# mks0601/ExAvatar_RELEASE

Measured on NVIDIA H100. Metric: avatar train-step frames/sec (fwd+bwd raster), higher is better.
Workload: dtype f32

## Files before the change

### exavatar_release_b200/csrc/composite_bwd4.cu

```cuda
#include "common.cuh"

namespace b2r {

constexpr int B4_THREADS = 64;
constexpr int B4_BATCH = 64;
#ifndef B4_QUEUE_DEPTH
#define B4_QUEUE_DEPTH 16
#endif
#ifndef B4_MIN_BLOCKS
#define B4_MIN_BLOCKS 10
#endif
constexpr int B4_QUEUE = B4_QUEUE_DEPTH;

struct B4Stage {
  float4 a[B4_BATCH];
  float4 b[B4_BATCH];
  float4 c[B4_BATCH];
};
constexpr int B4_GROUP = 4;
constexpr int B4_CQ = 32 + B4_GROUP;
struct B4Compact {
  float4 r[3][B4_CQ];
};
static_assert(B4_QUEUE % B4_GROUP == 0, "phase B runs when whole groups fill the transposition queue");

__device__ __forceinline__ float rcp_approx4(float x) {
  float y;
  asm("rcp.approx.ftz.f32 %0, %1;" : "=f"(y) : "f"(x));
  return y;
}

struct B4Smem {
  B4Stage stage[2];
  B4Compact compact[2];
  float2 tb[2][B4_QUEUE][33];
  float4 qm0[2][B4_QUEUE];
  float4 qm1[2][B4_QUEUE];
  float4 gpix[2][32];
  int warp_max_s[2];
};

template <bool HAS_DA>
__device__ __forceinline__ void bwd4_item(const B2RScene& sc, const Ctx& cx, const B2RBackwardArgs& args,
                                          float* __restrict__ gacc, B4Smem& sm, const int t_pos, const int seg,
                                          const int quad, const int n_multi) {
  B4Stage (&stage)[2] = sm.stage;
  B4Compact (&compact)[2] = sm.compact;
  float2 (&tb)[2][B4_QUEUE][33] = sm.tb;
  float4 (&qm0)[2][B4_QUEUE] = sm.qm0;
  float4 (&qm1)[2][B4_QUEUE] = sm.qm1;
  float4 (&gpix)[2][32] = sm.gpix;
  int (&warp_max_s)[2] = sm.warp_max_s;
  B2R_TRACE_BEGIN();
  const bool multi = t_pos < n_multi;
  const int tile = (int)cx.tile_order[t_pos];
  if (cx.skip_below && cx.tile_maxid[tile] < cx.skip_below) return;
  const int tx = tile % cx.gx, ty = tile / cx.gx;
  const int lane = threadIdx.x & 31, warp = threadIdx.x >> 5;
  const int W = sc.width, H = sc.height;
  const int wx0 = tx * TILE + (quad & 1) * 8, wy0 = ty * TILE + (quad >> 1) * 8 + warp * 4;
  if (wx0 >= W || ty * TILE + (quad >> 1) * 8 >= H) return;
  const int px = wx0 + (lane & 7), py = wy0 + (lane >> 3);
  const bool inside = px < W && py < H;
  const float pxf = (float)px, pyf = (float)py;
  const float rx0 = (float)wx0, ry0 = (float)wy0;
  const float rx1 = fminf((float)(wx0 + 7), (float)(W - 1)), ry1 = fminf((float)(wy0 + 3), (float)(H - 1));
  const size_t N = (size_t)W * H;
  const size_t pix = (size_t)py * W + px;

  const uint2 range = cx.ranges[tile];
  const int n = (int)(range.y - range.x);
  const int lo = multi ? seg * SEG : 0;
  const int hi = multi ? min(n, lo + SEG) : n;
  const uint32_t* ids = cx.dup_ids + range.x + lo;

  const int my_n = inside ? (int)cx.n_contrib[pix] : 0;
  const int my_hi = min(my_n, hi) - lo;
  const bool cont = my_n > hi;
  const float T_final = inside ? cx.final_T[pix] : 0.f;
  const float g_r = inside ? __ldg(args.dL_dcolor + pix) : 0.f;
  const float g_g = inside ? __ldg(args.dL_dcolor + N + pix) : 0.f;
  const float g_b = inside ? __ldg(args.dL_dcolor + 2 * N + pix) : 0.f;
  float g_d = 0.f, g_a = 0.f;
  if (HAS_DA && inside) {
    if (args.dL_ddepth) g_d = __ldg(args.dL_ddepth + pix);
    if (args.dL_dalpha) g_a = __ldg(args.dL_dalpha + pix);
  }
  const float* bgp = cx.bg ? cx.bg : sc.bg;
  const float Tfb = T_final * (__ldg(bgp) * g_r + __ldg(bgp + 1) * g_g + __ldg(bgp + 2) * g_b);
  gpix[warp][lane] = make_float4(g_r, g_g, g_b, g_d);

  const int warp_n = __reduce_max_sync(0xffffffffu, max(my_hi, 0));
  if (lane == 0) warp_max_s[warp] = warp_n;
  __syncthreads();
  const int nmax = max(warp_max_s[0], warp_max_s[1]);
  if (nmax == 0) {
    B2R_TRACE_END(0);
    return;
  }
  const int nb = (nmax + B4_BATCH - 1) / B4_BATCH;

  float T = T_final, B = 0.f;
  if (cont) {
    const int pit = (py - ty * TILE) * TILE + (px - tx * TILE);
    const int nrec = (n + SEG - 1) / SEG;
    const float* rec = cx.ckpt + (size_t)(cx.seg_start[t_pos] + seg) * CK_REC_FLOATS;
    const float* fin = cx.ckpt + (size_t)(cx.seg_start[t_pos] + nrec - 1) * CK_REC_FLOATS;
    const float4 c = __ldg(reinterpret_cast<const float4*>(rec) + pit);
    const float4 f = __ldg(reinterpret_cast<const float4*>(fin) + pit);
    float num = (f.y - c.y) * g_r + (f.z - c.z) * g_g + (f.w - c.w) * g_b;
    if (HAS_DA) {
      const float2 c2 = __ldg(reinterpret_cast<const float2*>(rec + CK_PLANE0) + pit);
      const float2 f2 = __ldg(reinterpret_cast<const float2*>(fin + CK_PLANE0) + pit);
      num += (f2.x - c2.x) * g_d + (f2.y - c2.y) * g_a;
    }
    T = c.x;
    B = __fdividef(num, c.x);
  }
  float la = 0.f, olm = 1.f, lv = 0.f;
  int qpos = 0;
  B4Compact& cw = compact[warp];
  const bool lane0 = lane == 0;
  const unsigned lanes_above = 0xfffffffeu << lane;
  const uint32_t first_grad = args.first_row;

  auto drain = [&](const int count) {
    constexpr int SHARE = 32 / B4_QUEUE;
    constexpr int ROWS = 4 / SHARE;
    static_assert(B4_QUEUE == 8 || B4_QUEUE == 16 || B4_QUEUE == 32, "queue depth");
    __syncwarp();
    const int h = lane & (B4_QUEUE - 1), part = lane / B4_QUEUE;
    const bool live = h < count;
    float Sx = 0.f, Sy = 0.f, Sxx = 0.f, Sxy = 0.f, Syy = 0.f, Sq = 0.f, Sr = 0.f, Sg = 0.f, Sb = 0.f, Sd = 0.f;
    float4 m0 = make_float4(0.f, 0.f, 0.f, 0.f), m1 = make_float4(0.f, 1.f, 0.f, 0.f);
    if (live) {
      m0 = qm0[warp][h];
      m1 = qm1[warp][h];
      const float mx = m0.x - rx0, my = m0.y - ry0;
      float dxs[8];
#pragma unroll
      for (int c = 0; c < 8; c++) dxs[c] = mx - (float)c;
#pragma unroll
      for (int r = 0; r < ROWS; r++) {
        const float dy = my - (float)(part * ROWS + r);
        float Rq = 0.f, Rx = 0.f, Rxx = 0.f;
#pragma unroll
        for (int c = 0; c < 8; c++) {
          const int p = (part * ROWS + r) * 8 + c;
          const float2 t = tb[warp][h][p];
          const float4 g = gpix[warp][p];
          const float hx = t.x * dxs[c];
          Rq += t.x;
          Rx += hx;
          Rxx = fmaf(hx, dxs[c], Rxx);
          Sr = fmaf(t.y, g.x, Sr);
          Sg = fmaf(t.y, g.y, Sg);
          Sb = fmaf(t.y, g.z, Sb);
          if (HAS_DA) Sd = fmaf(t.y, g.w, Sd);
        }
        const float hy = Rq * dy;
        Sq += Rq;
        Sx += Rx;
        Sxx += Rxx;
        Sy += hy;
        Syy = fmaf(hy, dy, Syy);
        Sxy = fmaf(Rx, dy, Sxy);
      }
    }
#pragma unroll
    for (int o = B4_QUEUE; o < 32; o <<= 1) {
      Sx += __shfl_xor_sync(0xffffffffu, Sx, o);
      Sy += __shfl_xor_sync(0xffffffffu, Sy, o);
      Sxx += __shfl_xor_sync(0xffffffffu, Sxx, o);
      Sxy += __shfl_xor_sync(0xffffffffu, Sxy, o);
      Syy += __shfl_xor_sync(0xffffffffu, Syy, o);
      Sq += __shfl_xor_sync(0xffffffffu, Sq, o);
      Sr += __shfl_xor_sync(0xffffffffu, Sr, o);
      Sg += __shfl_xor_sync(0xffffffffu, Sg, o);
      Sb += __shfl_xor_sync(0xffffffffu, Sb, o);
      if (HAS_DA) Sd += __shfl_xor_sync(0xffffffffu, Sd, o);
    }
    const uint32_t gid = __float_as_uint(m1.z) & 0x1fffffffu;
    if (live && part == 0 && gid >= first_grad) {
      float* dst = gacc + (size_t)gid * 12;
      red_add_v4(dst, 2.f * m0.z * Sx + m0.w * Sy, 2.f * m1.x * Sy + m0.w * Sx, Sxx, Sxy);
      red_add_v4(dst + 4, Syy, __fdividef(Sq, m1.y), Sd, 0.f);
      red_add_v4(dst + 8, Sr, Sg, Sb, 0.f);
    }
    __syncwarp();
  };

  const uint32_t id_begin = cx.id_begin, id_span = cx.id_span;
  uint32_t next_id = 0u;
  auto prefetch = [&](int b) {
    const int idx = b * B4_BATCH + threadIdx.x;
    next_id = idx < nmax ? __ldg(ids + idx) : 0u;
  };
  auto issue = [&](int b) {
    B4Stage& s = stage[b & 1];
    const int idx = b * B4_BATCH + threadIdx.x;
    if (idx < nmax) {
      const uint32_t id = next_id;
      if (id - id_begin < id_span) {
        const float4* src = reinterpret_cast<const float4*>(cx.geom + id);
        cp_async16(&s.a[threadIdx.x], src);
        cp_async16(&s.b[threadIdx.x], src + 1);
        cp_async16(&s.c[threadIdx.x], src + 2);
      } else {
        s.a[threadIdx.x] = make_float4(0.f, 0.f, -1.f, 0.f);
        s.b[threadIdx.x] = make_float4(-1.f, 0.f, 0.f, INFINITY);
      }
    }
    cp_async_commit();
  };

  auto replay_group = [&](const int k) {
    float araw[B4_GROUP], vv[B4_GROUP];
    bool valid[B4_GROUP];
#pragma unroll
    for (int u = 0; u < B4_GROUP; u++) {
      const float4 a = cw.r[0][k + u], bb = cw.r[1][k + u], col = cw.r[2][k + u];
      const float dx = a.x - pxf, dy = a.y - pyf;
      const float p2 = a.z * dx * dx + bb.x * dy * dy + a.w * dx * dy;
      araw[u] = bb.y * ex2_approx(p2);
      valid[u] = (__float_as_int(bb.w) < my_hi) && (p2 <= 0.f) && (araw[u] >= K_ALPHA_MIN);
      float v = fmaf(col.z, g_b, fmaf(col.y, g_g, col.x * g_r));
      if (HAS_DA) v += fmaf(bb.z, g_d, g_a);
      vv[u] = v;
      if (lane0) {
        qm0[warp][qpos + u] = a;
        qm1[warp][qpos + u] = make_float4(bb.x, bb.y, col.w, 0.f);
      }
    }
#pragma unroll
    for (int u = 0; u < B4_GROUP; u++) {
      const float ae = valid[u] ? fminf(K_ALPHA_MAX, araw[u]) : 0.f;
      const float om = 1.f - ae;
      const float rcp = rcp_approx4(om);
      const float Tn = T * rcp;
      B = fmaf(la, lv, olm * B);
      const float dLda = fmaf(vv[u] - B, Tn, -Tfb * rcp);
      la = ae; olm = om; lv = vv[u]; T = Tn;
      tb[warp][qpos + u][lane] = make_float2(valid[u] ? araw[u] * dLda : 0.f, ae * Tn);
    }
    qpos += B4_GROUP;
    if (qpos == B4_QUEUE) {
      drain(B4_QUEUE);
      qpos = 0;
    }
  };

  int head = 0, fill = 0;
  prefetch(nb - 1);
  issue(nb - 1);
  if (nb > 1) prefetch(nb - 2);
  for (int b = nb - 1; b >= 0; b--) {
    cp_async_wait<0>();
    __syncthreads();
    if (b > 0) {
      issue(b - 1);
      if (b > 1) prefetch(b - 2);
    }
    const int count = min(B4_BATCH, nmax - b * B4_BATCH);
    const B4Stage& s = stage[b & 1];
    if (warp_n <= b * B4_BATCH) continue;
    for (int c0 = ((count - 1) >> 5) << 5; c0 >= 0; c0 -= 32) {
      const int idx = c0 + lane;
      const int pos = b * B4_BATCH + idx;
      bool hit = false;
      float4 a, bb;
      if (idx < count && pos < warp_n) {
        a = s.a[idx];
        bb = s.b[idx];
        hit = !(region_max_p2(a.x, a.y, a.z, a.w, bb.x, rx0, ry0, rx1, ry1) < bb.w);
      }
      const unsigned mask = __ballot_sync(0xffffffffu, hit);
      if (mask == 0u) continue;
      if (hit) {
        int slot = head + fill + __popc(mask & lanes_above);
        slot -= slot >= B4_CQ ? B4_CQ : 0;
        cw.r[0][slot] = a;
        cw.r[1][slot] = make_float4(bb.x, bb.y, bb.z, __int_as_float(pos));
        cw.r[2][slot] = s.c[idx];
      }
      fill += __popc(mask);
      __syncwarp();
      for (; fill >= B4_GROUP; fill -= B4_GROUP) {
        replay_group(head);
        head = head + B4_GROUP == B4_CQ ? 0 : head + B4_GROUP;
      }
      __syncwarp();
    }
  }
  if (fill > 0) {
    if (lane >= fill && lane < B4_GROUP) {
      cw.r[0][head + lane] = make_float4(0.f, 0.f, 0.f, 0.f);
      cw.r[1][head + lane] = make_float4(0.f, 1.f, 0.f, __int_as_float(0x7fffffff));
      cw.r[2][head + lane] = make_float4(0.f, 0.f, 0.f, 0.f);
    }
    __syncwarp();
    replay_group(head);
  }
  if (qpos > 0) drain(qpos);
  if (threadIdx.x == 0) atomicAdd(reinterpret_cast<unsigned long long*>(&cx.status->consumed_bwd), (unsigned long long)nmax);
  B2R_TRACE_END(nmax);
}

template <bool HAS_DA>
__global__ void __launch_bounds__(B4_THREADS, B4_MIN_BLOCKS) composite_bwd4_kernel(const B2RScene sc, const Ctx cx,
                                                                    const B2RBackwardArgs args, float* __restrict__ gacc) {
  __shared__ B4Smem sm;
  const int n_multi = cx.ckpt ? (int)cx.classes[CLS_N_MULTI] : 0;
  const int total_segs = cx.ckpt ? (int)cx.classes[CLS_TOTAL_SEGS] : 0;
  const int items = 4 * (total_segs + (cx.tiles - n_multi));
  for (int item = blockIdx.x; item < items; item += gridDim.x) {
    const int s_item = item >> 2;
    int t_pos, seg;
    if (s_item < total_segs) {
      const uint2 e = cx.seg_table[s_item];
      t_pos = (int)e.x;
      seg = (int)e.y;
    } else {
      t_pos = n_multi + (s_item - total_segs);
      seg = 0;
    }
    bwd4_item<HAS_DA>(sc, cx, args, gacc, sm, t_pos, seg, item & 3, n_multi);
    __syncthreads();
  }
}

int launch_composite_bwd(const B2RScene& sc, const Ctx& cx, const B2RBackwardArgs& a, float* gacc, cudaStream_t st) {
  if (!(a.flags & B2R_BWD_SCRATCH_ZEROED)) cudaMemsetAsync(gacc, 0, (size_t)(sc.P > 0 ? sc.P : 1) * 12 * sizeof(float), st);
  const uint64_t extra = cx.ckpt ? cx.dup_capacity / SEG : 0;
  const uint64_t bound = 4ull * ((uint64_t)cx.tiles + extra);
  const uint64_t cap = (uint64_t)device_sm_count() * B4_MIN_BLOCKS * 4;
  const unsigned grid = (unsigned)(bound < cap ? bound : cap);
  ProfScope p(K_COMPOSITE_BWD, st);
  if (a.dL_ddepth || a.dL_dalpha)
    launch_k(composite_bwd4_kernel<true>, grid, B4_THREADS, 0, st, false, sc, cx, a, gacc);
  else
    launch_k(composite_bwd4_kernel<false>, grid, B4_THREADS, 0, st, false, sc, cx, a, gacc);
  return check_launch();
}

}

#ifdef B2R_CTA_TRACE
extern "C" int b2r_debug_trace_bwd(unsigned long long* buf) {
  return (int)cudaMemcpyToSymbol(b2r::g_cta_trace, &buf, sizeof(buf));
}
#endif
```

### exavatar_release_b200/csrc/composite_fwd4.cu

```cuda
#include "common.cuh"

namespace b2r {

#ifndef FL_BATCH_N
#define FL_BATCH_N 128
#endif
constexpr int F4_BATCH = 2 * FL_BATCH_N;
#ifndef F4_GROUP_N
#define F4_GROUP_N 4
#endif
constexpr int F4_GROUP = F4_GROUP_N;
constexpr int F4_CQ = 32 + F4_GROUP;

struct F4Stage {
  float4 a[F4_BATCH];
  float4 b[F4_BATCH];
  float4 c[F4_BATCH];
};
struct F4Queue {
  float4 r[3][F4_CQ];
};
struct Blend {
  float T, Tf, Cr, Cg, Cb, Dp, Aa;
  uint32_t last;
};
__device__ __forceinline__ bool alive(const Blend& s) { return s.T >= K_T_MIN; }

__device__ __forceinline__ void store4v(float* base, bool vec_ok, int lane, float v, bool inside) {
  if (vec_ok) {
    const float v1 = __shfl_down_sync(0xffffffffu, v, 1);
    const float v2 = __shfl_down_sync(0xffffffffu, v, 2);
    const float v3 = __shfl_down_sync(0xffffffffu, v, 3);
    if ((lane & 3) == 0 && inside) *reinterpret_cast<float4*>(base) = make_float4(v, v1, v2, v3);
  } else if (inside) {
    *base = v;
  }
}

__device__ __forceinline__ void blend_group4(const F4Queue& cw, const int k, Blend& s, const float pxf, const float pyf) {
  float al[F4_GROUP], om[F4_GROUP];
  bool ok[F4_GROUP];
  float4 col[F4_GROUP];
  float dep[F4_GROUP];
  uint32_t pos[F4_GROUP];
#pragma unroll
  for (int u = 0; u < F4_GROUP; u++) {
    const float4 a = cw.r[0][k + u], bb = cw.r[1][k + u];
    col[u] = cw.r[2][k + u];
    const float dx = a.x - pxf, dy = a.y - pyf;
    const float p2 = a.z * dx * dx + bb.x * dy * dy + a.w * dx * dy;
    const float ar = bb.y * ex2_approx(p2);
    al[u] = fminf(K_ALPHA_MAX, ar);
    ok[u] = (ar >= K_ALPHA_MIN) & (p2 <= 0.f);
    om[u] = ok[u] ? 1.f - al[u] : 1.f;
    dep[u] = bb.z;
    pos[u] = (uint32_t)__float_as_int(bb.w);
  }
#pragma unroll
  for (int u = 0; u < F4_GROUP; u++) {
    const float w = al[u] * s.T;
    const float Tn = s.T * om[u];
    const bool use = ok[u] & (Tn >= K_T_MIN);
    s.Cr = use ? fmaf(col[u].x, w, s.Cr) : s.Cr;
    s.Cg = use ? fmaf(col[u].y, w, s.Cg) : s.Cg;
    s.Cb = use ? fmaf(col[u].z, w, s.Cb) : s.Cb;
    s.Dp = use ? fmaf(dep[u], w, s.Dp) : s.Dp;
    s.Aa = use ? s.Aa + w : s.Aa;
    s.last = use ? pos[u] : s.last;
    s.Tf = use ? Tn : s.Tf;
    s.T = Tn;
  }
}

__device__ __forceinline__ void cull_and_blend(const F4Stage& st, const int idx, const bool in_range, const int pos1,
                                               F4Queue& cw, int& head, int& fill, Blend& s, const float rx0, const float ry0,
                                               const float rx1, const float ry1, const float pxf, const float pyf) {
  const int lane = threadIdx.x & 31;
  bool hit = false;
  float4 a, bb;
  if (in_range) {
    a = st.a[idx];
    bb = st.b[idx];
    hit = !(region_max_p2(a.x, a.y, a.z, a.w, bb.x, rx0, ry0, rx1, ry1) < bb.w);
  }
  const unsigned mask = __ballot_sync(0xffffffffu, hit);
  if (mask == 0u) return;
  if (hit) {
    int slot = head + fill + __popc(mask & ((1u << lane) - 1u));
    slot -= slot >= F4_CQ ? F4_CQ : 0;
    cw.r[0][slot] = a;
    cw.r[1][slot] = make_float4(bb.x, bb.y, bb.z, __int_as_float(pos1));
    cw.r[2][slot] = st.c[idx];
  }
  fill += __popc(mask);
  __syncwarp();
  for (; fill >= F4_GROUP; fill -= F4_GROUP) {
    blend_group4(cw, head, s, pxf, pyf);
    head = head + F4_GROUP == F4_CQ ? 0 : head + F4_GROUP;
  }
  __syncwarp();
}

__device__ __forceinline__ void flush_queue(F4Queue& cw, int& head, int& fill, Blend& s, const float pxf, const float pyf) {
  if (fill > 0) {
    const int lane = threadIdx.x & 31;
    if (lane >= fill && lane < F4_GROUP) {
      cw.r[0][head + lane] = make_float4(0.f, 0.f, 0.f, 0.f);
      cw.r[1][head + lane] = make_float4(0.f, 0.f, 0.f, 0.f);
      cw.r[2][head + lane] = make_float4(0.f, 0.f, 0.f, 0.f);
    }
    __syncwarp();
    blend_group4(cw, head, s, pxf, pyf);
    __syncwarp();
    head = head + F4_GROUP == F4_CQ ? 0 : head + F4_GROUP;
    fill = 0;
  }
}

__device__ __forceinline__ void store_checkpoint(float* rec, const int pix_in_tile, const Blend& s) {
  reinterpret_cast<float4*>(rec)[pix_in_tile] = make_float4(s.Tf, s.Cr, s.Cg, s.Cb);
  reinterpret_cast<float2*>(rec + CK_PLANE0)[pix_in_tile] = make_float2(s.Dp, s.Aa);
}

__device__ __forceinline__ void write_outputs(const B2RScene& sc, const Ctx& cx, const B2RForwardOutputs& out, const int vec_ok,
                                              const Blend& S, const int px, const int py, const bool inside, const int lane) {
  const float T = S.Tf;
  const size_t N = (size_t)sc.width * sc.height;
  const size_t pix = (size_t)py * sc.width + px;
  const float* bgp = cx.bg ? cx.bg : sc.bg;
  const float bg0 = __ldg(bgp), bg1 = __ldg(bgp + 1), bg2 = __ldg(bgp + 2);
  const bool v = vec_ok != 0;
  store4v(out.color + pix, v, lane, fmaf(T, bg0, S.Cr), inside);
  store4v(out.color + N + pix, v, lane, fmaf(T, bg1, S.Cg), inside);
  store4v(out.color + 2 * N + pix, v, lane, fmaf(T, bg2, S.Cb), inside);
  store4v(out.depth + pix, v, lane, S.Dp, inside);
  store4v(out.alpha + pix, v, lane, S.Aa, inside);
  store4v(cx.final_T + pix, v, lane, T, inside);
  store4v(reinterpret_cast<float*>(cx.n_contrib) + pix, v, lane, __uint_as_float(S.last), inside);
}

constexpr int FL_THREADS = 64;
constexpr int FL_BATCH = FL_BATCH_N;
static_assert(SEG % FL_BATCH == 0, "checkpoint cuts fall on batch boundaries");

#ifndef F4_MIN_BLOCKS
#define F4_MIN_BLOCKS 14
#endif
__global__ void __launch_bounds__(FL_THREADS, F4_MIN_BLOCKS) composite_fwd_kernel(const B2RScene sc, const Ctx cx,
                                                                          const B2RForwardOutputs out, const int vec_ok) {
  __shared__ F4Stage stage_raw;
  __shared__ F4Queue queue[2];
  B2R_TRACE_BEGIN();
  const int lane = threadIdx.x & 31, warp = threadIdx.x >> 5;
  const int W = sc.width, H = sc.height;
  const int t_pos = blockIdx.x >> 2;
  const int tile = (int)cx.tile_order[t_pos];
  if (cx.skip_below && cx.tile_maxid[tile] < cx.skip_below) return;
  const int quad = blockIdx.x & 3;
  const int tx = tile % cx.gx, ty = tile / cx.gx;
  const int wx0 = tx * TILE + (quad & 1) * 8, wy0 = ty * TILE + (quad >> 1) * 8 + warp * 4;
  if (wx0 >= W || ty * TILE + (quad >> 1) * 8 >= H) return;
  const int px = wx0 + (lane & 7), py = wy0 + (lane >> 3);
  const bool inside = px < W && py < H;
  const float pxf = (float)px, pyf = (float)py;
  const float rx0 = (float)wx0, ry0 = (float)wy0;
  const float rx1 = fminf((float)(wx0 + 7), (float)(W - 1)), ry1 = fminf((float)(wy0 + 3), (float)(H - 1));
  const int pix_in_tile = (py - ty * TILE) * TILE + (px - tx * TILE);

  const uint2 range = cx.ranges[tile];
  const int n = (int)(range.y - range.x);
  const uint32_t* ids = cx.dup_ids + range.x;
  const int nb = (n + FL_BATCH - 1) / FL_BATCH;
  const int nrec = (n + SEG - 1) / SEG;
  float* ck = nullptr;
  if (cx.ckpt && t_pos < (int)cx.classes[CLS_N_MULTI]) ck = cx.ckpt + (size_t)cx.seg_start[t_pos] * CK_REC_FLOATS;

  const uint32_t id_begin = cx.id_begin, id_span = cx.id_span;
  constexpr int FL_PER_THREAD = FL_BATCH / FL_THREADS;
  uint32_t next_id[FL_PER_THREAD];
  auto prefetch = [&](int b) {
#pragma unroll
    for (int u = 0; u < FL_PER_THREAD; u++) {
      const int idx = b * FL_BATCH + threadIdx.x + u * FL_THREADS;
      next_id[u] = idx < n ? __ldg(ids + idx) : 0u;
    }
  };
  auto issue = [&](int b) {
    const int half = (b & 1) * FL_BATCH;
#pragma unroll
    for (int u = 0; u < FL_PER_THREAD; u++) {
      const int slot = half + threadIdx.x + u * FL_THREADS;
      const int idx = b * FL_BATCH + threadIdx.x + u * FL_THREADS;
      if (idx < n) {
        const uint32_t id = next_id[u];
        if (id - id_begin < id_span) {
          const float4* src = reinterpret_cast<const float4*>(cx.geom + id);
          cp_async16(&stage_raw.a[slot], src);
          cp_async16(&stage_raw.b[slot], src + 1);
          cp_async16(&stage_raw.c[slot], src + 2);
        } else {
          stage_raw.a[slot] = make_float4(0.f, 0.f, -1.f, 0.f);
          stage_raw.b[slot] = make_float4(-1.f, 0.f, 0.f, INFINITY);
        }
      }
    }
    cp_async_commit();
  };

  Blend S;
  S.T = S.Tf = inside ? 1.f : 0.f;
  S.Cr = S.Cg = S.Cb = S.Dp = S.Aa = 0.f;
  S.last = 0;
  F4Queue& cw = queue[warp];
  int head = 0, fill = 0, staged = 0;
  if (nb > 0) {
    prefetch(0);
    issue(0);
    if (nb > 1) prefetch(1);
  }
  for (int b = 0; b < nb; b++) {
    cp_async_wait<0>();
    if (__syncthreads_and(!alive(S))) break;
    if (b + 1 < nb) {
      issue(b + 1);
      if (b + 2 < nb) prefetch(b + 2);
    }
    const int count = min(FL_BATCH, n - b * FL_BATCH);
    staged += count;
    const int half = (b & 1) * FL_BATCH;
    bool warp_live = __any_sync(0xffffffffu, alive(S));
    for (int c0 = 0; c0 < count && warp_live; c0 += 32) {
      const int idx = c0 + lane;
      cull_and_blend(stage_raw, half + idx, idx < count, b * FL_BATCH + idx + 1, cw, head, fill, S, rx0, ry0, rx1, ry1, pxf, pyf);
      warp_live = __any_sync(0xffffffffu, alive(S));
    }
    if (ck && ((b + 1) * FL_BATCH) % SEG == 0 && b + 1 < nb) {
      flush_queue(cw, head, fill, S, pxf, pyf);
      if (inside) store_checkpoint(ck + (size_t)((b + 1) * FL_BATCH / SEG - 1) * CK_REC_FLOATS, pix_in_tile, S);
    }
  }
  flush_queue(cw, head, fill, S, pxf, pyf);
  cp_async_wait<0>();
  if (ck && nrec >= 2 && inside) store_checkpoint(ck + (size_t)(nrec - 1) * CK_REC_FLOATS, pix_in_tile, S);
  if (threadIdx.x == 0 && staged)
    atomicAdd(reinterpret_cast<unsigned long long*>(&cx.status->consumed_fwd), 2ull * (unsigned long long)staged);
  write_outputs(sc, cx, out, vec_ok, S, px, py, inside, lane);
  B2R_TRACE_END(n);
}

int launch_composite_fwd(const B2RScene& sc, const Ctx& cx, const B2RForwardOutputs& out, cudaStream_t st) {
  auto al16 = [](const void* p) { return (reinterpret_cast<uintptr_t>(p) & 15) == 0; };
  const int vec_ok = (sc.width % 4 == 0) && al16(out.color) && al16(out.depth) && al16(out.alpha) && al16(cx.final_T) &&
                     al16(cx.n_contrib);
  ProfScope p(K_COMPOSITE_FWD, st);
  launch_k(composite_fwd_kernel, (unsigned)(cx.tiles * 4), FL_THREADS, 0, st, false, sc, cx, out, vec_ok);
  return check_launch();
}

}

#ifdef B2R_CTA_TRACE
extern "C" int b2r_debug_trace_fwd(unsigned long long* buf) {
  return (int)cudaMemcpyToSymbol(b2r::g_cta_trace, &buf, sizeof(buf));
}
#endif
```

Measured before the change: 1893.

## Track in-view staged gaussians with ballot bitmasks and generalize forward staging ring

Both composite kernels stop writing sentinel float4 values for out-of-view or out-of-range gaussians. Instead they record a per-warp ballot bitmask of valid entries in shared memory, and the cull loop skips whole 32-entry chunks whose mask is zero. The forward kernel's double buffer becomes a configurable ring with a partial cp.async wait, and ids are loaded one stage ahead. With the default depth of 2 the pipeline stays equivalent, so the main runtime effect is fewer shared stores and skipped empty chunks, at the cost of an extra ballot per issue.

Measured after the change: 1896, median of 6. No clear change (+0.1%).

```diff
diff --git a/exavatar_release_b200/csrc/composite_bwd4.cu b/exavatar_release_b200/csrc/composite_bwd4.cu
--- a/exavatar_release_b200/csrc/composite_bwd4.cu
+++ b/exavatar_release_b200/csrc/composite_bwd4.cu
@@ -16,6 +16,7 @@
   float4 a[B4_BATCH];
   float4 b[B4_BATCH];
   float4 c[B4_BATCH];
+  uint32_t in_view[B4_BATCH / 32];
 };
 constexpr int B4_GROUP = 4;
 constexpr int B4_CQ = 32 + B4_GROUP;
@@ -198,19 +199,15 @@
   };
   auto issue = [&](int b) {
     B4Stage& s = stage[b & 1];
-    const int idx = b * B4_BATCH + threadIdx.x;
-    if (idx < nmax) {
-      const uint32_t id = next_id;
-      if (id - id_begin < id_span) {
-        const float4* src = reinterpret_cast<const float4*>(cx.geom + id);
-        cp_async16(&s.a[threadIdx.x], src);
-        cp_async16(&s.b[threadIdx.x], src + 1);
-        cp_async16(&s.c[threadIdx.x], src + 2);
-      } else {
-        s.a[threadIdx.x] = make_float4(0.f, 0.f, -1.f, 0.f);
-        s.b[threadIdx.x] = make_float4(-1.f, 0.f, 0.f, INFINITY);
-      }
-    }
+    const bool in_view = b * B4_BATCH + (int)threadIdx.x < nmax && next_id - id_begin < id_span;
+    if (in_view) {
+      const float4* src = reinterpret_cast<const float4*>(cx.geom + next_id);
+      cp_async16(&s.a[threadIdx.x], src);
+      cp_async16(&s.b[threadIdx.x], src + 1);
+      cp_async16(&s.c[threadIdx.x], src + 2);
+    }
+    const unsigned word = __ballot_sync(0xffffffffu, in_view);
+    if (lane0) s.in_view[warp] = word;
     cp_async_commit();
   };
 
@@ -265,11 +262,13 @@
     const B4Stage& s = stage[b & 1];
     if (warp_n <= b * B4_BATCH) continue;
     for (int c0 = ((count - 1) >> 5) << 5; c0 >= 0; c0 -= 32) {
+      const uint32_t word = s.in_view[c0 >> 5];
+      if (word == 0u) continue;
       const int idx = c0 + lane;
       const int pos = b * B4_BATCH + idx;
       bool hit = false;
       float4 a, bb;
-      if (idx < count && pos < warp_n) {
+      if (((word >> lane) & 1u) && pos < warp_n) {
         a = s.a[idx];
         bb = s.b[idx];
         hit = !(region_max_p2(a.x, a.y, a.z, a.w, bb.x, rx0, ry0, rx1, ry1) < bb.w);
diff --git a/exavatar_release_b200/csrc/composite_fwd4.cu b/exavatar_release_b200/csrc/composite_fwd4.cu
--- a/exavatar_release_b200/csrc/composite_fwd4.cu
+++ b/exavatar_release_b200/csrc/composite_fwd4.cu
@@ -5,7 +5,12 @@
 #ifndef FL_BATCH_N
 #define FL_BATCH_N 128
 #endif
-constexpr int F4_BATCH = 2 * FL_BATCH_N;
+#ifndef F4_STAGES_N
+#define F4_STAGES_N 2
+#endif
+constexpr int F4_STAGES = F4_STAGES_N;
+constexpr int F4_BATCH = F4_STAGES * FL_BATCH_N;
+static_assert(F4_STAGES >= 2 && (F4_STAGES & (F4_STAGES - 1)) == 0, "ring depth: a power of two >= 2");
 #ifndef F4_GROUP_N
 #define F4_GROUP_N 4
 #endif
@@ -16,6 +21,7 @@
   float4 a[F4_BATCH];
   float4 b[F4_BATCH];
   float4 c[F4_BATCH];
+  uint32_t in_view[F4_BATCH / 32];
 };
 struct F4Queue {
   float4 r[3][F4_CQ];
@@ -72,13 +78,13 @@
   }
 }
 
-__device__ __forceinline__ void cull_and_blend(const F4Stage& st, const int idx, const bool in_range, const int pos1,
+__device__ __forceinline__ void cull_and_blend(const F4Stage& st, const int idx, const bool in_view, const int pos1,
                                                F4Queue& cw, int& head, int& fill, Blend& s, const float rx0, const float ry0,
                                                const float rx1, const float ry1, const float pxf, const float pyf) {
   const int lane = threadIdx.x & 31;
   bool hit = false;
   float4 a, bb;
-  if (in_range) {
+  if (in_view) {
     a = st.a[idx];
     bb = st.b[idx];
     hit = !(region_max_p2(a.x, a.y, a.z, a.w, bb.x, rx0, ry0, rx1, ry1) < bb.w);
@@ -142,6 +148,7 @@
 constexpr int FL_THREADS = 64;
 constexpr int FL_BATCH = FL_BATCH_N;
 static_assert(SEG % FL_BATCH == 0, "checkpoint cuts fall on batch boundaries");
+static_assert(FL_BATCH % FL_THREADS == 0, "every thread gathers the same number of entries per batch");
 
 #ifndef F4_MIN_BLOCKS
 #define F4_MIN_BLOCKS 14
@@ -177,31 +184,28 @@
 
   const uint32_t id_begin = cx.id_begin, id_span = cx.id_span;
   constexpr int FL_PER_THREAD = FL_BATCH / FL_THREADS;
-  uint32_t next_id[FL_PER_THREAD];
-  auto prefetch = [&](int b) {
+  auto load_ids = [&](int b, uint32_t (&dst)[FL_PER_THREAD]) {
 #pragma unroll
     for (int u = 0; u < FL_PER_THREAD; u++) {
       const int idx = b * FL_BATCH + threadIdx.x + u * FL_THREADS;
-      next_id[u] = idx < n ? __ldg(ids + idx) : 0u;
+      dst[u] = idx < n ? __ldg(ids + idx) : 0u;
     }
   };
-  auto issue = [&](int b) {
-    const int half = (b & 1) * FL_BATCH;
-#pragma unroll
-    for (int u = 0; u < FL_PER_THREAD; u++) {
-      const int slot = half + threadIdx.x + u * FL_THREADS;
-      const int idx = b * FL_BATCH + threadIdx.x + u * FL_THREADS;
-      if (idx < n) {
-        const uint32_t id = next_id[u];
-        if (id - id_begin < id_span) {
-          const float4* src = reinterpret_cast<const float4*>(cx.geom + id);
+  auto issue = [&](int b, const uint32_t (&id)[FL_PER_THREAD]) {
+    if (b < nb) {
+      const int ring = (int)((unsigned)b % F4_STAGES) * FL_BATCH;
+#pragma unroll
+      for (int u = 0; u < FL_PER_THREAD; u++) {
+        const int slot = ring + threadIdx.x + u * FL_THREADS;
+        const bool in_view = b * FL_BATCH + threadIdx.x + u * FL_THREADS < n && id[u] - id_begin < id_span;
+        if (in_view) {
+          const float4* src = reinterpret_cast<const float4*>(cx.geom + id[u]);
           cp_async16(&stage_raw.a[slot], src);
           cp_async16(&stage_raw.b[slot], src + 1);
           cp_async16(&stage_raw.c[slot], src + 2);
-        } else {
-          stage_raw.a[slot] = make_float4(0.f, 0.f, -1.f, 0.f);
-          stage_raw.b[slot] = make_float4(-1.f, 0.f, 0.f, INFINITY);
         }
+        const unsigned word = __ballot_sync(0xffffffffu, in_view);
+        if (lane == 0) stage_raw.in_view[slot >> 5] = word;
       }
     }
     cp_async_commit();
@@ -213,25 +217,30 @@
   S.last = 0;
   F4Queue& cw = queue[warp];
   int head = 0, fill = 0, staged = 0;
-  if (nb > 0) {
-    prefetch(0);
-    issue(0);
-    if (nb > 1) prefetch(1);
+  uint32_t next_id[FL_PER_THREAD];
+  {
+    uint32_t first[F4_STAGES - 1][FL_PER_THREAD];
+#pragma unroll
+    for (int j = 0; j < F4_STAGES - 1; j++) load_ids(j, first[j]);
+    load_ids(F4_STAGES - 1, next_id);
+#pragma unroll
+    for (int j = 0; j < F4_STAGES - 1; j++) issue(j, first[j]);
   }
   for (int b = 0; b < nb; b++) {
-    cp_async_wait<0>();
+    cp_async_wait<F4_STAGES - 2>();
     if (__syncthreads_and(!alive(S))) break;
-    if (b + 1 < nb) {
-      issue(b + 1);
-      if (b + 2 < nb) prefetch(b + 2);
-    }
+    issue(b + F4_STAGES - 1, next_id);
+    load_ids(b + F4_STAGES, next_id);
     const int count = min(FL_BATCH, n - b * FL_BATCH);
     staged += count;
-    const int half = (b & 1) * FL_BATCH;
+    const int ring = (int)((unsigned)b % F4_STAGES) * FL_BATCH;
     bool warp_live = __any_sync(0xffffffffu, alive(S));
     for (int c0 = 0; c0 < count && warp_live; c0 += 32) {
+      const uint32_t word = stage_raw.in_view[(ring + c0) >> 5];
+      if (word == 0u) continue;
       const int idx = c0 + lane;
-      cull_and_blend(stage_raw, half + idx, idx < count, b * FL_BATCH + idx + 1, cw, head, fill, S, rx0, ry0, rx1, ry1, pxf, pyf);
+      cull_and_blend(stage_raw, ring + idx, (word >> lane) & 1u, b * FL_BATCH + idx + 1, cw, head, fill, S, rx0, ry0, rx1,
+                     ry1, pxf, pyf);
       warp_live = __any_sync(0xffffffffu, alive(S));
     }
     if (ck && ((b + 1) * FL_BATCH) % SEG == 0 && b + 1 < nb) {
```
